# cristianpjensen/thesis-pai-reconstruction

Measured on AMD Instinct MI355X. Metric: train images/sec (256x256, bs=64) Pix2Pix step, higher is better.
Workload: dtype bf16; 1 GPU; Pix2Pix generator+PatchGAN GAN step, 256x256x1 pairs, 64 images/GPU (BASELINE configs[1]); global_batch=64, per_gpu_batch=64, loss_type=gan, parallelism=dp1, grad_bucket_dtype=f32

## Files before the change

include/pai_hip.h:

```cpp
#ifndef PAI_HIP_H
#define PAI_HIP_H

#include <stdint.h>

#ifdef __cplusplus
extern "C" {
#endif

#define PAI_F32 0
#define PAI_BF16 1
#define PAI_U8 2

#define PAI_ACT_NONE 0
#define PAI_ACT_LRELU 1
#define PAI_ACT_RELU 2
#define PAI_ACT_TANH 3
#define PAI_ACT_SILU 4

const char* pai_last_error(void);
int pai_version(void);
int pai_build_flags(void);
int pai_device_info(int* cu_count, int* lds_bytes, char* arch_name, int arch_name_len);

#define PAI_TUNABLE_UNSET (-2147483647 - 1)
// ... 32 lines not shown
int pai_handle_set_wgrad_workspace(void* handle, void* device_memory, int64_t bytes);

int pai_set_workspace(void* zeroed_device_memory, int64_t bytes);
int64_t pai_conv_workspace_bytes(const pai_conv_desc* d, int op);
int pai_set_scratch(void* device_memory, int64_t bytes);
int64_t pai_conv_scratch_bytes(const pai_conv_desc* d, int op);
int pai_set_wgrad_workspace(void* device_memory, int64_t bytes);
int64_t pai_conv_wgrad_workspace_bytes(const pai_conv_desc* d);

int pai_conv_fwd(const pai_conv_desc* d, const void* x1, const void* x2, const void* w_fwd,
                 const float* bias, void* y_raw, void* y_act, float* y_f32, float* stats,
                 void* stream);

int pai_conv_dgrad(const pai_conv_desc* d, const void* dy, const void* w_dgrad, void* dx1,
                   void* dx2, int only_c2, void* stream);

int pai_conv_dgrad_act(const pai_conv_desc* d, const void* dy, const void* w_dgrad, void* dx1,
                       void* dx2, const void* a1, int act1, void* stream);

typedef struct pai_bwd_epilogue {
    const void* z;
    const void* add;
    const float* scale;
    const float* shift;
    const float* mean;
    const float* rstd;
    float* partials;
    int32_t act1, act2;
} pai_bwd_epilogue;
int pai_conv_dgrad_bn_rows_max(const pai_conv_desc* d);
// ... 118 lines not shown
int pai_gate_apply_bwd(int dtype, const void* dout, const void* x, const float* att, const float* logit,
                       int64_t M, int C, const float* mean_a, const float* rstd_a, void* dx_skip, float* dl,
                       float* partials, int relu_out, void* stream);
int pai_gate_hidden_bwd(int dtype, const float* dl, const float* logit, const void* h, const void* ig,
                        const void* sg, int64_t M, int K, const float* mean_a, const float* rstd_a,
                        const float* gamma_a, const float* sums_a, const float* w_a, const float* mean_i,
                        const float* rstd_i, const float* mean_s, const float* rstd_s, void* dsum,
                        float* partials_i, float* partials_s, float* dw_a, float* db_a, void* stream);

int pai_bce_logits(const float* logits, int64_t numel, float target, float loss_scale,
                   double* loss, float grad_scale, float* grad, void* stream);
int pai_l1(const float* pred, const float* target, int64_t numel, float loss_scale, double* loss,
           float grad_scale, float* grad, void* stream);
int pai_mse(const float* pred, const float* target, int64_t numel, float loss_scale, double* loss,
            float grad_scale, float* grad, void* stream);
int pai_scalar_take(double* acc, float* out, void* stream);
int pai_metrics_take(double* sums, int64_t n_images, int64_t numel, float* out3, void* stream);
int pai_tanh_bwd(int dtype, const float* pred, const float* g_a, const float* g_b, int64_t numel,
                 void* dh, void* stream);

int pai_denormalize(const float* x, const float* grad_out_or_null, int64_t numel, float* out,
                    void* stream);

int pai_ssim_sse(const float* pred, const float* target, int NC, int H, int W, int denorm,
                 double* out2, double* per_image, float* full_map, void* stream);
int pai_ssim_psnr_bwd(const float* pred, const float* target, int NC, int H, int W, int denorm,
                      float w_ssim, float w_psnr, const double* sse, float* grad, float* workspace,
                      void* stream);
int64_t pai_ssim_bwd_workspace_floats(int NC, int H, int W);
int pai_eval_planes(const float* pred, const float* target, int NC, int H, int W, int denorm,
// ... 90 lines not shown
```

thesis-pai-reconstruction_amd/build.py:

```python
from __future__ import annotations

import os
import subprocess
import sys
from concurrent.futures import ThreadPoolExecutor

HERE = os.path.dirname(os.path.abspath(__file__))
CSRC = os.path.join(HERE, "csrc")
LIB = os.path.join(HERE, "libpai_hip.so")
STAMPS = os.path.join(CSRC, ".build_stamps.json")
SOURCES = ["api.hip", "gg_simt.hip", "gg_mfma.hip", "gg_wg3.hip", "gg_thin.hip", "gg_small.hip", "gg_group.hip", "gg_pw.hip", "bn.hip", "ew_stream.hip", "gate.hip", "resnet.hip", "inorm.hip", "vit.hip", "loss.hip", "ssim.hip", "eval.hip", "misc.hip", "comm.hip", "plan.hip", "data.hip", "palette.hip", "film_norm.hip"]
HEADERS = [os.path.join(CSRC, "common.h"), os.path.join(CSRC, "plan.h"), os.path.join(CSRC, "gg_tile.h"), os.path.join(HERE, "..", "include", "pai_hip.h")]
FLAGS = ["-O3", "--offload-arch=gfx950", "-fPIC", "-std=c++17", "-Wall", "-Wno-unused-function",
         "-fno-gpu-rdc", "-mllvm", "-amdgpu-mfma-vgpr-form=1"]
EXTRA_FLAGS = {"gg_mfma.hip": ["-fno-slp-vectorize"]}


def _hipcc():
    for c in (os.environ.get("HIPCC"), "/opt/rocm/bin/hipcc", "hipcc"):
        if c and (os.path.isabs(c) and os.path.exists(c) or not os.path.isabs(c)):
            return c
    raise RuntimeError("hipcc not found")


def _digest(paths, extra=""):
    import hashlib
# ... 58 lines not shown
```

thesis-pai-reconstruction_amd/csrc/api.hip:

```cpp
#include <stdarg.h>

#include "common.h"

static thread_local char g_err[512] = "";

void pai_set_error(const char* fmt, ...) {
    va_list ap;
    va_start(ap, fmt);
    vsnprintf(g_err, sizeof(g_err), fmt, ap);
    va_end(ap);
}

extern "C" const char* pai_last_error(void) { return g_err; }
extern "C" int pai_version(void) { return 139; }

extern "C" int pai_build_flags(void) { return 0; }

extern "C" int pai_device_info(int* cu_count, int* lds_bytes, char* arch_name, int arch_name_len) {
    int dev = 0;
    hipError_t e = hipGetDevice(&dev);
    PAI_CHECK(e == hipSuccess, "hipGetDevice: %s", hipGetErrorString(e));
    hipDeviceProp_t p;
    e = hipGetDeviceProperties(&p, dev);
    PAI_CHECK(e == hipSuccess, "hipGetDeviceProperties: %s", hipGetErrorString(e));
    if (cu_count) *cu_count = p.multiProcessorCount;
    if (lds_bytes) *lds_bytes = (int)p.sharedMemPerBlock;
    if (arch_name && arch_name_len > 0) {
        strncpy(arch_name, p.gcnArchName, arch_name_len - 1);
        arch_name[arch_name_len - 1] = 0;
// ... 560 lines not shown
extern "C" int pai_conv_dgrad(const pai_conv_desc* d, const void* dy, const void* w_dgrad,
                              void* dx1, void* dx2, int only_c2, void* stream) {
    GG g;
    if (gg_build_dgrad(d, &g)) return 1;
    PAI_CHECK(dy && w_dgrad, "pai_conv_dgrad: null dy / w");
    PAI_CHECK(only_c2 ? (dx2 && d->C2 > 0) : (dx1 != nullptr), "pai_conv_dgrad: missing output");
    PAI_CHECK(d->C2 == 0 || dx2, "pai_conv_dgrad: C2 > 0 but dx2 is null");
    FwdArgs a;
    memset(&a, 0, sizeof(a));
    a.x1 = dy; a.w = w_dgrad;
    a.y1 = dx1; a.y2 = dx2;
    a.skip_d1 = only_c2;
    return run_fwd(d->dtype, g, a, (hipStream_t)stream);
}

extern "C" int pai_conv_dgrad_act(const pai_conv_desc* d, const void* dy, const void* w_dgrad,
                                  void* dx1, void* dx2, const void* a1, int act1, void* stream) {
    GG g;
    if (gg_build_dgrad(d, &g)) return 1;
    PAI_CHECK(dy && w_dgrad && dx1 && a1, "pai_conv_dgrad_act: null pointer");
    PAI_CHECK(d->C2 == 0 || dx2, "pai_conv_dgrad_act: C2 > 0 but dx2 is null");
    PAI_CHECK(act1 == PAI_ACT_LRELU || act1 == PAI_ACT_RELU || act1 == PAI_ACT_NONE, "pai_conv_dgrad_act: act1=%d", act1);
    FwdArgs a;
    memset(&a, 0, sizeof(a));
    a.x1 = dy; a.w = w_dgrad;
    a.y1 = dx1; a.y2 = dx2;
    hipStream_t s = (hipStream_t)stream;
    FwdPick p = pick_fwd(d->dtype, g, a);
    const bool fused = p.fused || p.k == FK_HEAD_DGRAD;
    if (fused) {
// ... 179 lines not shown
```

thesis-pai-reconstruction_amd/csrc/common.h:

```cpp
#pragma once
#include <hip/hip_runtime.h>
#include <stdint.h>
#include <stdio.h>
#include <string.h>

#include "../../include/pai_hip.h"
#include "plan.h"

typedef unsigned short bf16_t;

void pai_set_error(const char* fmt, ...);

#define PAI_CHECK(cond, ...)                 \
    do {                                     \
        if (!(cond)) {                       \
            pai_set_error(__VA_ARGS__);      \
            return 1;                        \
        }                                    \
    } while (0)

#define PAI_LAUNCH_CHECK()                                              \
    do {                                                                \
        hipError_t e_ = hipGetLastError();                              \
        if (e_ != hipSuccess) {                                         \
// ... 209 lines not shown
int small_rows(const GG& g);
int launch_small(const GG& g, const FwdArgs& a, hipStream_t s);
bool grouped3_ok(int dtype, const GG& g, const FwdArgs& a);
int grouped3_rows(const GG& g);
int launch_grouped3(const GG& g, const FwdArgs& a, hipStream_t s);

bool thin_fwd_ok(int dtype, const GG& g, const FwdArgs& a);
bool thin_dgrad_ok(int dtype, const GG& g, const FwdArgs& a);
bool thin_dgrad_shape_ok(int dtype, const GG& g);
int64_t thin_dgrad_scratch_bytes(const GG& g, const FwdArgs& a);
int launch_thin_fwd(const GG& g, const FwdArgs& a, hipStream_t s);
bool head_dgrad_ok(int dtype, const GG& g, const FwdArgs& a);
int launch_head_dgrad(const GG& g, const FwdArgs& a, hipStream_t s);
int thin_fwd_bwd_rows(int dtype, const GG& g, const FwdArgs& a, int act1, const void* add, const float* scale);
int launch_thin_dgrad(const GG& g, const FwdArgs& a, hipStream_t s);

struct WgradArgs {
    const void *x1, *x2, *dy;
    float* dw;
    float* dbias;
    int overwrite;
    int overwrite_bias;
    float* slab;
    const float *pscale, *pshift;
    int pact;
};
float* wgrad_slab_acquire(int64_t bytes);
int launch_wgrad_slab_sum(float* dw, const float* slab, int nsplits, int64_t n, int overwrite, hipStream_t s);
bool grouped3_wgrad_ok(int dtype, const GG& g, const float* dbias);
int64_t grouped3_wgrad_part_bytes(const GG& g);
// ... 24 lines not shown
```

thesis-pai-reconstruction_amd/csrc/gg_thin.hip:

```cpp
#include "common.h"

#ifndef THIN_ABL
#define THIN_ABL 0
#endif
typedef __attribute__((ext_vector_type(8))) __bf16 bf8_t;
typedef __attribute__((ext_vector_type(4))) __bf16 bf4_t;
typedef __attribute__((ext_vector_type(4))) float f4_t;
typedef __attribute__((ext_vector_type(8))) short s8_t;
typedef __attribute__((ext_vector_type(8))) unsigned short us8_t;

__device__ uint4 g_zero_line_thin[16];


__device__ __forceinline__ bf8_t relu8(bf8_t f) {
    s8_t x = __builtin_bit_cast(s8_t, f);
    const s8_t z = {0, 0, 0, 0, 0, 0, 0, 0};
    return __builtin_bit_cast(bf8_t, __builtin_elementwise_max(x, z));
}

template <int S>
__device__ __forceinline__ us8_t thin_gather8(__amdgpu_buffer_rsrc_t rs, int e0, int ix0, int TW, bool valid) {
    typedef __attribute__((ext_vector_type(4))) unsigned u4_t;
    const int base = ix0 & ~1, o = ix0 & 1;
    const bool neg = valid && e0 + base < 0;
// ... 714 lines not shown
        const int oyl = i >> 5, oxl = i & 31;
        const int oy = 2 * ty0 + oyl, ox = 2 * tx0 + oxl;
        const int ph = (oyl & 1) * 2 + (oxl & 1);
        const int hy0 = (oyl >> 1) + 1, hx0 = (oxl >> 1) + 1;
        const size_t o = ((size_t)n * g.OH + oy) * g.OW + ox;
#pragma unroll
        for (int tt = 0; tt < T; ++tt) {
            const int t = t0 + tt;
            float v = a.bias ? a.bias[t] : 0.f;
#pragma unroll
            for (int k = 0; k < 4; ++k) {
                const int e = tab[ph][k];
                const int hy = hy0 + (int)(signed char)(e & 0xff), hx = hx0 + (int)(signed char)((e >> 8) & 0xff);
                v += Ys[tt][hy * TU_HW + hx][(e >> 16) & 0xff];
            }
            if (t < g.D1) {
                if (a.y1 && !a.skip_d1) ((bf16_t*)a.y1)[o * g.D1 + t] = f2bf(v);
            } else if (a.y2) {
                ((bf16_t*)a.y2)[o * g.D2 + (t - g.D1)] = f2bf(v);
            }
            if (a.yact || a.yf32) {
                const float av = act_apply(v, a.eact);
                if (a.yact) ((bf16_t*)a.yact)[o * g.Cout + t] = f2bf(av);
                if (a.yf32) a.yf32[o * g.Cout + t] = av;
            }
        }
    }
}

static bool thin_up_ok(const GG& g) {
    return pai_tunable("thin_up", 1) && g.nphase == 4 && g.ntaps == 4 && g.OS == 2 && g.wtaps == 16 && (g.H % 16) == 0 &&
           (g.W % 16) == 0 && (g.Cin == 64 || g.Cin == 128);
}

int launch_thin_dgrad(const GG& g, const FwdArgs& a, hipStream_t s) {
    const int T = thin_dgrad_T(g, a);
    const int t0 = (g.Cout == 2 && a.skip_d1) ? 1 : 0;
    if (thin_up_ok(g)) {
        const int tx = g.W / 16, ty = g.H / 16;
        const dim3 grid(g.N * tx * ty);
        if (T == 1 && g.Cin == 128) PAI_LAUNCH((thin_up_k<1, 4>), grid, dim3(256), 0, s, g, a, t0, tx, ty);
        else if (T == 1) PAI_LAUNCH((thin_up_k<1, 2>), grid, dim3(256), 0, s, g, a, t0, tx, ty);
        else if (g.Cin == 128) PAI_LAUNCH((thin_up_k<2, 4>), grid, dim3(256), 0, s, g, a, t0, tx, ty);
        else PAI_LAUNCH((thin_up_k<2, 2>), grid, dim3(256), 0, s, g, a, t0, tx, ty);
        PAI_LAUNCH_CHECK();
        return 0;
    }
// ... 416 lines not shown
```

thesis-pai-reconstruction_amd/engine.py:

```python
from __future__ import annotations

import os
from typing import Callable, List, Optional

import torch
import torch.nn as nn

from . import ops
from .ops import ACT_LRELU, ACT_NONE, ACT_RELU, ACT_TANH

BN_EPS_DEFAULT = 1e-5


def _fwd_pack_strides(mod) -> tuple:
    if isinstance(mod, nn.ConvTranspose2d):
        cin, cout, kh, kw = mod.weight.shape
        return (1, kh * kw * cin, kw * cin, cin)
    cout, cin, kh, kw = mod.weight.shape
    return (kh * kw * cin, 1, kw * cin, cin)


def _strides_match(t: torch.Tensor, want: tuple) -> bool:
    return all(s == w or n == 1 for s, w, n in zip(t.stride(), want, t.shape))

# ... 759 lines not shown
        S["logits"] = torch.empty(N, 1, P["oh"], P["ow"], dtype=torch.float32, device=device)
        S["grads"] = None
        return S

    def release(self, S):
        S["P"]["free"].append(S)

    def _to_nhwc(self, t, dst, dtype):
        t = t.to(torch.float32)
        t = t.contiguous() if t.shape[1] == 1 else t.permute(0, 2, 3, 1).contiguous()
        if dtype == torch.float32:
            return t.reshape(-1)
        ops.cast(t, dst)
        return dst

    def forward(self, x, y, dtype, y2=None):
        if not (x.is_cuda and y.is_cuda):
            raise ops.PaiError("Discriminator (HIP) needs HIP device tensors; there is no CPU path")
        N, C, H, W = x.shape
        if C != self.in_ch or y.shape != x.shape or (y2 is not None and y2.shape != x.shape):
            raise ops.PaiError(f"Discriminator expects [N,{self.in_ch},H,W] tensors of one shape, got {tuple(x.shape)} "
                               f"and {tuple(y.shape)}")
        reps = 1 if y2 is None else 2
        S = self.acquire(N * reps, H, W, dtype, x.device)
        P = S["P"]
        if y2 is None and dtype != torch.float32 and C == 1:
            ops.cast_multi([(x.detach().to(torch.float32).contiguous().reshape(-1), S["x"]),
                            (y.detach().to(torch.float32).contiguous().reshape(-1), S["y"])])
            S["xin"], S["yin"] = S["x"], S["y"]
        elif y2 is None:
            S["xin"] = self._to_nhwc(x, S["x"], dtype)
# ... 1 lines not shown
        else:
            half = N * H * W * C
            pairs = []
            for src, dst in ((x, S["x"][:half]), (x, S["x"][half:]), (y, S["y"][:half]), (y2, S["y"][half:])):
                t = src.detach().to(torch.float32)
                t = t.contiguous() if C == 1 else t.permute(0, 2, 3, 1).contiguous()
                pairs.append((t.reshape(-1), dst))
            ops.cast_multi(pairs)
            S["xin"], S["yin"] = S["x"], S["y"]
        refresh_packs(self.packs, dtype)
        wf, _ = self.packs[0].get(dtype)
        ops.conv_fwd(P["desc"][0], S["xin"], S["yin"], wf, self.convs[0].bias, y_act=S["a"][0])
        for k in range(1, 4):
            wf, _ = self.packs[k].get(dtype)
            ops.conv_fwd(P["desc"][k], S["a"][k - 1], None, wf, self.convs[k].bias, y_act=S["a"][k])
        wf, _ = self.packs[4].get(dtype)
        S["logits"] = torch.empty_like(S["logits"])
        ops.conv_fwd(P["desc"][4], S["a"][3], None, wf, None, y_f32=S["logits"])
        return S["logits"], S

    def _wgrad_desc(self, P, k):
        if os.environ.get("PAI_D_WGRAD_SOLO", "1") in ("", "0"):
            return P["desc"][k]
        solo = P.setdefault("desc_solo", {})
        if k not in solo:
            import copy
            d = copy.copy(P["desc"][k])
            d.hints = 1
            solo[k] = d
        return solo[k]

    def backward(self, S, glogits, need_params: bool, need_dy: bool, fresh: bool = False):
        conv_wgrad = ops.conv_wgrad_overwrite_w if fresh else ops.conv_wgrad
        P = S["P"]
        N, H, W, dtype, dev = P["N"], P["H"], P["W"], P["dtype"], P["device"]
        if S["grads"] is None:
            G = {"du": [torch.empty_like(a) for a in S["a"]],
                 "dl": torch.empty(S["logits"].numel(), dtype=dtype, device=dev),
                 "dy": torch.empty(N * H * W * self.in_ch, dtype=dtype, device=dev)}
            S["grads"] = G
        G = S["grads"]
        A = self.arena() if need_params else None
        hook = self.grad_ready_hook
        glogits = glogits.contiguous().float()
        if dtype == torch.float32:
            dl = glogits.reshape(-1)
        else:
            ops.cast(glogits, G["dl"])
            dl = G["dl"]
        d = P["desc"][4]
        side = self._side
        if need_params:
            with torch.cuda.stream(side.fork(d)):
                ops.conv_wgrad(d, S["a"][3], None, dl, A.seg(self.convs[4].weight), None)
                if hook is not None:
                    hook(A, A.end_of(self.convs[4].weight))
            side.mark_scratch()
        _, wd = self.packs[4].get(dtype)
        ops.conv_dgrad_act(d, dl, wd, G["du"][3], None, S["a"][3], ACT_LRELU)
        for k in range(3, -1, -1):
            conv = self.convs[k]
            d = P["desc"][k]
            if need_params and k == 0:
                with torch.cuda.stream(side.fork_tail()):
                    (ops.conv_wgrad if min(_cin_cout(conv)) <= 2 else conv_wgrad)(
                        d, S["xin"], S["yin"], G["du"][0], A.seg(conv.weight), A.seg(conv.bias))
            elif need_params:
                with torch.cuda.stream(side.fork(d)):
                    conv_wgrad(self._wgrad_desc(P, k), S["a"][k - 1], None, G["du"][k], A.seg(conv.weight), A.seg(conv.bias))
                    if hook is not None:
                        hook(A, A.end_of(conv.bias))
            if k > 0:
                _, wd = self.packs[k].get(dtype)
                ops.conv_dgrad_act(d, G["du"][k], wd, G["du"][k - 1], None, S["a"][k - 1], ACT_LRELU)
            elif need_dy:
                _, wd = self.packs[0].get(dtype)
                ops.conv_dgrad(d, G["du"][0], wd, None, G["dy"], only_c2=True)
        side.join()
        if need_params and hook is not None:
            hook(A, A.end_of(self.convs[0].bias))
        if not need_dy:
            return None
        gy = torch.empty(N * H * W * self.in_ch, dtype=torch.float32, device=dev)
        ops.cast(G["dy"], gy)
        if self.in_ch == 1:
            return gy.view(N, 1, H, W)
        return gy.view(N, H, W, self.in_ch).permute(0, 3, 1, 2)
```

thesis-pai-reconstruction_amd/functional.py:

```python
from __future__ import annotations

import math

import torch

from . import ops


class _SlotRef:

    def __init__(self, engine, slot):
        self.engine, self.slot = engine, slot

    def take(self):
        if self.slot is None:
            raise ops.PaiError("second backward through the same forward: the engine's activation slot has already "
                               "been consumed (retain_graph is not supported)")
        slot, self.slot = self.slot, None
        return slot

    def __del__(self):
        if self.slot is not None:
            try:
                self.engine.release(self.slot)
# ... 71 lines not shown
        else:
            engine.release(slot)
        return logits

    @staticmethod
    def backward(ctx, glogits):
        engine, slot, params = ctx.engine, ctx.ref.take(), ctx.params
        arena = engine.arena()
        fresh = arena.begin_backward(params, overwrite_weights=True)
        engine.backward(slot, glogits, True, False, fresh)
        arena.attach(params)
        engine.release(slot)
        return (None,) * (5 + len(params))


class DiscGenLossFunction(torch.autograd.Function):

    @staticmethod
    def forward(ctx, x, pred, target, engine, dtype, l1_weight, *params):
        _check_f32_cuda(x, pred, target)
        if ctx.needs_input_grad[0] or ctx.needs_input_grad[2]:
            raise ops.PaiError("gradient w.r.t. the conditioning image / the target is not supported")
        logits, slot = engine.forward(x, pred, dtype)
        pc, tc = pred.contiguous().float(), target.contiguous().float()
        need_pred, need_params = ctx.needs_input_grad[1], any(ctx.needs_input_grad[6:])
        need = need_pred or need_params
        gl = torch.empty_like(logits) if need else None
        gp = torch.empty_like(pc) if need_pred else None
        ent = _ACC.get(pc.device, "gan_g")
        ops.bce_logits(logits, 1.0, 1.0, ent[0], 1.0, gl)
        ops.l1(pc, tc, float(l1_weight), ent[0], float(l1_weight), gp)
        out = torch.empty((), dtype=torch.float32, device=pc.device)
        ops.scalar_take(ent[0], out)
        _ACC.taken(ent)
        if need:
            ctx.engine, ctx.ref, ctx.params = engine, _SlotRef(engine, slot), params
            ctx.need_pred, ctx.need_params = need_pred, need_params
            ctx.save_for_backward(*[g for g in (gl, gp) if g is not None])
        else:
            engine.release(slot)
        return out

    @staticmethod
    def backward(ctx, gout):
        engine, slot, params = ctx.engine, ctx.ref.take(), ctx.params
        saved = list(ctx.saved_tensors)
        gl = _scaled(saved.pop(0), gout)
        fresh = False
        if ctx.need_params:
            arena = engine.arena()
            fresh = arena.begin_backward(params, overwrite_weights=True)
        gy = engine.backward(slot, gl, ctx.need_params, ctx.need_pred, fresh)
        if ctx.need_params:
            arena.attach(params)
        engine.release(slot)
        if ctx.need_pred:
            gp = _scaled(saved.pop(0), gout)
            if gy.is_contiguous() and gy.numel() % 8 == 0:
                ops.add_act(torch.float32, gy, gp, ops.ACT_NONE, gy)
            else:
                gy = gy + gp
        return (None, gy, None, None, None, None) + (None,) * len(params)


def _check_f32_cuda(*ts):
    for t in ts:
        if not t.is_cuda:
            raise ops.PaiError("pai losses/metrics need HIP device tensors (no CPU fallback exists)")


class _MeanLoss(torch.autograd.Function):
# ... 39 lines not shown
        ent[1] = False


_ACC = _Accumulators()


_UNIT = {}


def unit_seed(device) -> torch.Tensor:
    t = _UNIT.get(device.index)
    if t is None:
        t = torch.ones((), dtype=torch.float32, device=device)
        _UNIT[device.index] = t
    return t


def _scaled(grad, gout):
    u = _UNIT.get(gout.device.index) if gout.is_cuda else None
    if u is not None and gout.data_ptr() == u.data_ptr():
        return grad
    return grad * gout


class _GanDiscLoss(torch.autograd.Function):

    @staticmethod
    def forward(ctx, labels, n_real):
        _check_f32_cuda(labels)
        x = labels.contiguous().float()
# ... 324 lines not shown
```

thesis-pai-reconstruction_amd/lib.py:

```python
from __future__ import annotations

import ctypes as C
import os

HERE = os.path.dirname(os.path.abspath(__file__))
LIB_PATH = os.environ.get("PAI_HIP_LIB") or os.path.join(HERE, "libpai_hip.so")

F32, BF16 = 0, 1
U8 = 2
ACT_NONE, ACT_LRELU, ACT_RELU, ACT_TANH = 0, 1, 2, 3
ACT_SILU = 4
HINT_SOLO = 1


class PaiError(RuntimeError):
    pass


class ConvDesc(C.Structure):
    _fields_ = [("dtype", C.c_int32), ("transposed", C.c_int32),
                ("N", C.c_int32), ("H", C.c_int32), ("W", C.c_int32),
                ("C1", C.c_int32), ("C2", C.c_int32), ("Cout", C.c_int32),
                ("kernel", C.c_int32), ("stride", C.c_int32), ("pad", C.c_int32),
                ("relu1", C.c_int32), ("relu2", C.c_int32), ("epilogue_act", C.c_int32),
# ... 33 lines not shown
    "pai_conv_out_hw": (_I, [_D, C.POINTER(_I), C.POINTER(_I)]),
    "pai_conv_fwd_stats_rows": (_I, [_D]),
    "pai_conv_fwd_stats_rows_max": (_I, [_D]),
    "pai_bn_stats_buffer_rows": (_I, [_I]),
    "pai_conv_kernel_id": (_I, [_D, _I]),
    "pai_conv_kernel_name": (_I, [_D, _I, C.c_char_p, _I]),
    "pai_set_workspace": (_I, [_P, _L]),
    "pai_conv_workspace_bytes": (_L, [_D, _I]),
    "pai_set_scratch": (_I, [_P, _L]),
    "pai_conv_scratch_bytes": (_L, [_D, _I]),
    "pai_set_wgrad_workspace": (_I, [_P, _L]),
    "pai_conv_wgrad_workspace_bytes": (_L, [_D]),
    "pai_conv_fwd": (_I, [_D, _P, _P, _P, _P, _P, _P, _P, _P, _P]),
    "pai_conv_dgrad": (_I, [_D, _P, _P, _P, _P, _I, _P]),
    "pai_conv_dgrad_act": (_I, [_D, _P, _P, _P, _P, _P, _I, _P]),
    "pai_conv_dgrad_bn_rows_max": (_I, [_D]),
    "pai_conv_dgrad_bn": (_I, [_D, _P, _P, _P, _P, C.POINTER(BwdEpilogue), C.POINTER(_I), _P]),
    "pai_bn_bwd_finalize": (_I, [_P, _I, _I, _P, _P, _P, _P]),
    "pai_conv_fwd_bn": (_I, [_D, _P, _P, _P, _P, _P, _P, _I, C.POINTER(BnTrain), _P, _P]),
    "pai_conv_dgrad_bn_apply": (_I, [_D, _P, _P, _P, _P, C.POINTER(BwdEpilogue), _P, _P, _P, _P, _P, _P]),
    "pai_conv_bn_fused": (_I, [_D, _I]),
    "pai_conv_wgrad": (_I, [_D, _P, _P, _P, _P, _P, _P]),
    "pai_conv_wgrad_overwrite": (_I, [_D, _P, _P, _P, _P, _P, _P]),
    "pai_conv_wgrad_overwrite_w": (_I, [_D, _P, _P, _P, _P, _P, _P]),
    "pai_conv_prologue_ok": (_I, [_D]),
    "pai_conv_fwd_pro": (_I, [_D, _P, _P, _P, _P, _P, _P, _P, _I, _P]),
    "pai_conv_wgrad_pro": (_I, [_D, _P, _P, _P, _P, _I, _P, _P, _I, _P]),
    "pai_pack_weights": (_I, [_I, _P, _I, _I, _I, _P, _P, _P]),
    "pai_build_flags": (_I, []),
    "pai_pack_weights_multi": (_I, [_I, _P, _P, _P, _P, _P, _P, _P]),
# ... 130 lines not shown
```

thesis-pai-reconstruction_amd/models/wrapper.py:

```python
from typing import Literal

import torch
import torch.nn as nn

from .. import functional as PF
from .. import ops
from ..engine import DiscEngine
from ..lightning import LightningModule
from .utils import denormalize, init_weights, psnr, rmse, ssim

L1_WEIGHT = 50


class UnetWrapper(LightningModule):

    def __init__(self, unet: nn.Module,
                 loss_type: Literal["gan", "ssim", "psnr", "ssim+psnr", "mse"] = "gan"):
        super().__init__()
        self.automatic_optimization = False
        self.unet = unet
        self.loss_type = loss_type
        self.reuse_generator_forward = True

        self.discriminator = None
# ... 73 lines not shown
        metrics_early = None

        if self.loss_type == "gan":
            opt_d = self.optimizers()[1]
            if reuse:
                self.unet.bn_updates_per_forward = 2
                try:
                    pred_g = self.unet(x)
                finally:
                    self.unet.bn_updates_per_forward = 1

                metrics_early = self._metrics_async(pred_g, target)

            self.toggle_optimizer(opt_d)
            pred = pred_g.detach() if reuse else self.unet(x)
            if getattr(self.discriminator, "supports_batched_pairs", False):
                n = x.shape[0]
                labels = self.discriminator.forward_pairs(x, target, pred)
                d_loss = PF.gan_discriminator_loss_pairs(labels, n)
            else:
                target_label = self.discriminator(x, target)
                pred_label = self.discriminator(x, pred)
                d_loss = self.discriminator_loss(pred_label, target_label)
            self.log("d_loss", d_loss, prog_bar=True)
            self.discriminator.zero_grad(set_to_none=True)
            self._arm(opt_d)
            self.manual_backward(d_loss)
            opt_d.step()
            self.untoggle_optimizer(opt_d)

        opt_g = self.optimizers()
# ... 54 lines not shown
            h = nnops.ConvK4S2.apply(h, conv.weight, conv.bias, ACT_NONE, dtype)
            h = nnops.InstanceNormAct.apply(h, float(norm.eps), ACT_LRELU)
        else:
            h = nnops.ConvK4S2.apply(h, conv.weight, conv.bias, ACT_LRELU, dtype)
        return h.float().permute(0, 3, 1, 2)


class Discriminator(nn.Module):

    def __init__(self, in_channels: int = 3):
        super().__init__()
        self.in_channels = in_channels
        self.compute_dtype = torch.float32
        self.supports_batched_pairs = True
        self.supports_fused_generator_loss = True
        self.discriminator = nn.Sequential(
            DiscriminatorBlock(in_channels * 2, 64, norm=False),
            DiscriminatorBlock(64, 128),
            DiscriminatorBlock(128, 256),
            DiscriminatorBlock(256, 512),
            nn.Conv2d(512, 1, kernel_size=4, padding=1, bias=False),
        )
        self._engine = None

    @property
    def engine(self) -> DiscEngine:
        if self._engine is None:
            object.__setattr__(self, "_engine", DiscEngine(self))
        return self._engine

    def forward(self, x, y):
        eng = self.engine
        params = [p for p, _ in eng.ordered_params()]
        return PF.DiscFunction.apply(x, y, eng, self.compute_dtype, *params)

    def generator_loss(self, x, y, target, l1_weight):
        eng = self.engine
        params = [p for p, _ in eng.ordered_params()]
        return PF.DiscGenLossFunction.apply(x, y, target, eng, self.compute_dtype, float(l1_weight), *params)

    def forward_pairs(self, x, y_real, y_fake):
        eng = self.engine
        params = [p for p, _ in eng.ordered_params()]
        return PF.DiscPairsFunction.apply(x.detach(), y_real.detach(), y_fake.detach(), eng, self.compute_dtype, *params)
```

thesis-pai-reconstruction_amd/ops.py:

```python
from __future__ import annotations

import ctypes as C

import threading
from typing import Optional

import torch

from . import lib as L
from .lib import ACT_LRELU, ACT_NONE, ACT_RELU, ACT_SILU, ACT_TANH, BF16, F32, U8, ConvDesc, PaiError


def code_of(dtype: torch.dtype) -> int:
    if dtype == torch.float32:
        return F32
    if dtype == torch.bfloat16:
        return BF16
    raise PaiError(f"unsupported storage dtype {dtype}")


_TLS = threading.local()


def _stream():
# ... 271 lines not shown
        L.check(L.load().pai_conv_wgrad_pro(C.byref(d), _p(x1), _p(dy), _p(dw, torch.float32), _p(dbias, torch.float32),
                                            int(overwrite), _p(pre_scale, torch.float32), _p(pre_shift, torch.float32),
                                            int(pre_act), _stream()), "pai_conv_wgrad_pro")


def conv_dgrad(d, dy, w_dgrad, dx1, dx2=None, only_c2=False):
    with _Timed(d, 1):
        L.check(L.load().pai_conv_dgrad(C.byref(d), _p(dy), _p(w_dgrad), _p(dx1), _p(dx2), int(only_c2),
                                        _stream()), "pai_conv_dgrad")


def conv_dgrad_act(d, dy, w_dgrad, dx1, dx2, a1, act1):
    with _Timed(d, 1):
        L.check(L.load().pai_conv_dgrad_act(C.byref(d), _p(dy), _p(w_dgrad), _p(dx1), _p(dx2), _p(a1), int(act1),
                                            _stream()), "pai_conv_dgrad_act")


def conv_dgrad_bn_rows_max(d) -> int:
    return L.load().pai_conv_dgrad_bn_rows_max(C.byref(d))


def conv_dgrad_bn(d, dy, w_dgrad, dx1, dx2, z, act1, add=None, act2=ACT_NONE, scale=None, shift=None,
                  mean=None, rstd=None, partials=None) -> int:
    e = L.BwdEpilogue(_p(z), _p(add), _p(scale, torch.float32), _p(shift, torch.float32), _p(mean, torch.float32),
                      _p(rstd, torch.float32), _p(partials, torch.float32), int(act1), int(act2))
    rows = C.c_int(0)
    with _Timed(d, 1):
        L.check(L.load().pai_conv_dgrad_bn(C.byref(d), _p(dy), _p(w_dgrad), _p(dx1), _p(dx2), C.byref(e),
                                           C.byref(rows), _stream()), "pai_conv_dgrad_bn")
    return rows.value
# ... 761 lines not shown
```

Before: 11470 images/s.

## Fuse discriminator head conv, BCE loss, and head dgrad into one kernel

```diff
diff --git a/include/pai_hip.h b/include/pai_hip.h
--- a/include/pai_hip.h
+++ b/include/pai_hip.h
@@ -70,6 +70,10 @@
 
 int pai_conv_dgrad(const pai_conv_desc* d, const void* dy, const void* w_dgrad, void* dx1,
                    void* dx2, int only_c2, void* stream);
+
+int pai_conv_dgrad_f32add_ok(const pai_conv_desc* d);
+int pai_conv_dgrad_f32add(const pai_conv_desc* d, const void* dy, const void* w_dgrad, const float* addend,
+                          float* dx2_f32, void* stream);
 
 int pai_conv_dgrad_act(const pai_conv_desc* d, const void* dy, const void* w_dgrad, void* dx1,
                        void* dx2, const void* a1, int act1, void* stream);
@@ -218,6 +222,10 @@
            float grad_scale, float* grad, void* stream);
 int pai_mse(const float* pred, const float* target, int64_t numel, float loss_scale, double* loss,
             float grad_scale, float* grad, void* stream);
+int pai_head_loss_ok(const pai_conv_desc* d, int has_bias);
+int pai_head_loss(const pai_conv_desc* d, const void* a3, const void* w_fwd, const void* w_dgrad, int n_first,
+                  float target_first, float target_rest, float loss_scale, double* loss, float grad_scale,
+                  float* logits, void* dl, float* dl_f32, void* du, const void* act_src, int act, void* stream);
 int pai_scalar_take(double* acc, float* out, void* stream);
 int pai_metrics_take(double* sums, int64_t n_images, int64_t numel, float* out3, void* stream);
 int pai_tanh_bwd(int dtype, const float* pred, const float* g_a, const float* g_b, int64_t numel,
diff --git a/thesis-pai-reconstruction_amd/build.py b/thesis-pai-reconstruction_amd/build.py
--- a/thesis-pai-reconstruction_amd/build.py
+++ b/thesis-pai-reconstruction_amd/build.py
@@ -9,7 +9,7 @@
 CSRC = os.path.join(HERE, "csrc")
 LIB = os.path.join(HERE, "libpai_hip.so")
 STAMPS = os.path.join(CSRC, ".build_stamps.json")
-SOURCES = ["api.hip", "gg_simt.hip", "gg_mfma.hip", "gg_wg3.hip", "gg_thin.hip", "gg_small.hip", "gg_group.hip", "gg_pw.hip", "bn.hip", "ew_stream.hip", "gate.hip", "resnet.hip", "inorm.hip", "vit.hip", "loss.hip", "ssim.hip", "eval.hip", "misc.hip", "comm.hip", "plan.hip", "data.hip", "palette.hip", "film_norm.hip"]
+SOURCES = ["api.hip", "gg_simt.hip", "gg_mfma.hip", "gg_wg3.hip", "gg_thin.hip", "head.hip", "gg_small.hip", "gg_group.hip", "gg_pw.hip", "bn.hip", "ew_stream.hip", "gate.hip", "resnet.hip", "inorm.hip", "vit.hip", "loss.hip", "ssim.hip", "eval.hip", "misc.hip", "comm.hip", "plan.hip", "data.hip", "palette.hip", "film_norm.hip"]
 HEADERS = [os.path.join(CSRC, "common.h"), os.path.join(CSRC, "plan.h"), os.path.join(CSRC, "gg_tile.h"), os.path.join(HERE, "..", "include", "pai_hip.h")]
 FLAGS = ["-O3", "--offload-arch=gfx950", "-fPIC", "-std=c++17", "-Wall", "-Wno-unused-function",
          "-fno-gpu-rdc", "-mllvm", "-amdgpu-mfma-vgpr-form=1"]
diff --git a/thesis-pai-reconstruction_amd/csrc/api.hip b/thesis-pai-reconstruction_amd/csrc/api.hip
--- a/thesis-pai-reconstruction_amd/csrc/api.hip
+++ b/thesis-pai-reconstruction_amd/csrc/api.hip
@@ -12,7 +12,7 @@
 }
 
 extern "C" const char* pai_last_error(void) { return g_err; }
-extern "C" int pai_version(void) { return 139; }
+extern "C" int pai_version(void) { return 140; }
 
 extern "C" int pai_build_flags(void) { return 0; }
 
@@ -603,6 +603,26 @@
     return run_fwd(d->dtype, g, a, (hipStream_t)stream);
 }
 
+extern "C" int pai_conv_dgrad_f32add_ok(const pai_conv_desc* d) {
+    GG g;
+    if (!d || gg_build_dgrad(d, &g)) return 0;
+    return pai_tunable("head_fused", 1) && thin_up_f32add_ok(d->dtype, g) ? 1 : 0;
+}
+
+extern "C" int pai_conv_dgrad_f32add(const pai_conv_desc* d, const void* dy, const void* w_dgrad, const float* addend,
+                                     float* dx2_f32, void* stream) {
+    GG g;
+    if (gg_build_dgrad(d, &g)) return 1;
+    PAI_CHECK(dy && w_dgrad && addend && dx2_f32, "pai_conv_dgrad_f32add: null pointer");
+    PAI_CHECK(thin_up_f32add_ok(d->dtype, g), "pai_conv_dgrad_f32add: not a bf16 (1 | 1)-channel k4 s2 layer on thin_up_k (ask pai_conv_dgrad_f32add_ok)");
+    FwdArgs a;
+    memset(&a, 0, sizeof(a));
+    a.x1 = dy; a.w = w_dgrad;
+    a.yf32 = dx2_f32; a.badd = addend;
+    a.skip_d1 = 1;
+    return launch_thin_dgrad(g, a, (hipStream_t)stream);
+}
+
 extern "C" int pai_conv_dgrad_act(const pai_conv_desc* d, const void* dy, const void* w_dgrad,
                                   void* dx1, void* dx2, const void* a1, int act1, void* stream) {
     GG g;
diff --git a/thesis-pai-reconstruction_amd/csrc/common.h b/thesis-pai-reconstruction_amd/csrc/common.h
--- a/thesis-pai-reconstruction_amd/csrc/common.h
+++ b/thesis-pai-reconstruction_amd/csrc/common.h
@@ -247,6 +247,7 @@
 int launch_head_dgrad(const GG& g, const FwdArgs& a, hipStream_t s);
 int thin_fwd_bwd_rows(int dtype, const GG& g, const FwdArgs& a, int act1, const void* add, const float* scale);
 int launch_thin_dgrad(const GG& g, const FwdArgs& a, hipStream_t s);
+bool thin_up_f32add_ok(int dtype, const GG& g);
 
 struct WgradArgs {
     const void *x1, *x2, *dy;
diff --git a/thesis-pai-reconstruction_amd/csrc/gg_thin.hip b/thesis-pai-reconstruction_amd/csrc/gg_thin.hip
--- a/thesis-pai-reconstruction_amd/csrc/gg_thin.hip
+++ b/thesis-pai-reconstruction_amd/csrc/gg_thin.hip
@@ -752,6 +752,13 @@
                 const int hy = hy0 + (int)(signed char)(e & 0xff), hx = hx0 + (int)(signed char)((e >> 8) & 0xff);
                 v += Ys[tt][hy * TU_HW + hx][(e >> 16) & 0xff];
             }
+            if (a.badd) {
+                if (t >= g.D1) {
+                    const size_t idx = o * g.D2 + (t - g.D1);
+                    a.yf32[idx] = bf2f(f2bf(v)) + ((const float*)a.badd)[idx];
+                }
+                continue;
+            }
             if (t < g.D1) {
                 if (a.y1 && !a.skip_d1) ((bf16_t*)a.y1)[o * g.D1 + t] = f2bf(v);
             } else if (a.y2) {
@@ -769,6 +776,10 @@
 static bool thin_up_ok(const GG& g) {
     return pai_tunable("thin_up", 1) && g.nphase == 4 && g.ntaps == 4 && g.OS == 2 && g.wtaps == 16 && (g.H % 16) == 0 &&
            (g.W % 16) == 0 && (g.Cin == 64 || g.Cin == 128);
+}
+
+bool thin_up_f32add_ok(int dtype, const GG& g) {
+    return thin_dgrad_shape_ok(dtype, g) && thin_up_ok(g) && g.Cout == 2 && g.D1 == 1 && g.D2 == 1;
 }
 
 int launch_thin_dgrad(const GG& g, const FwdArgs& a, hipStream_t s) {
diff --git a/thesis-pai-reconstruction_amd/csrc/head.hip b/thesis-pai-reconstruction_amd/csrc/head.hip
--- /dev/null
+++ b/thesis-pai-reconstruction_amd/csrc/head.hip
@@ -0,0 +1,209 @@
+#include "common.h"
+
+typedef __attribute__((ext_vector_type(8))) __bf16 bf8_t;
+typedef __attribute__((ext_vector_type(4))) float f4_t;
+
+constexpr int HL_THREADS = 512, HL_WAVES = HL_THREADS / 64;
+constexpr int HL_LD = 17;
+constexpr int64_t HL_LDS_MAX = 96 * 1024;
+
+struct HeadLoss {
+    const bf16_t* a3;
+    const bf16_t* wf;
+    const bf16_t* wd;
+    float* logits;
+    bf16_t* dl;
+    float* dl32;
+    bf16_t* du;
+    const bf16_t* act_src;
+    double* loss;
+    int N, H, W, C, OH, OW;
+    int n_first;
+    float t_first, t_rest;
+    double ls_first, ls_rest;
+    float gs_first, gs_rest;
+    int act;
+    int rg;
+    int xcd;
+};
+
+static int64_t head_loss_lds_bytes(int H, int W, int C, bool with_du) {
+    const int64_t ys = (((int64_t)H * W * HL_LD * 4) + 15) & ~(int64_t)15;
+    const int64_t dls = (((int64_t)(H - 1) * (W - 1) * 4) + 15) & ~(int64_t)15;
+    return ys + dls + (with_du ? (int64_t)16 * C * 2 : 0);
+}
+
+template <int KS>
+__global__ __launch_bounds__(HL_THREADS) void head_loss_k(HeadLoss p) {
+    extern __shared__ __attribute__((aligned(16))) unsigned char hl_sm[];
+    __shared__ double wsum[HL_WAVES];
+    const int P = p.H * p.W, Q = p.OH * p.OW;
+    float* Ys = (float*)hl_sm;
+    float* dls = (float*)(hl_sm + ((((size_t)P * HL_LD * 4) + 15) & ~(size_t)15));
+    bf16_t* wt = (bf16_t*)((unsigned char*)dls + ((((size_t)Q * 4) + 15) & ~(size_t)15));
+    const int tid = threadIdx.x, lane = tid & 63, wid = tid >> 6;
+    const int fr = lane & 15, fq = lane >> 4;
+    int n, rg;
+    if (p.xcd) {
+        n = (blockIdx.x & 7) + 8 * (blockIdx.x / (8 * p.rg));
+        rg = (blockIdx.x >> 3) % p.rg;
+    } else {
+        n = blockIdx.x / p.rg;
+        rg = blockIdx.x - n * p.rg;
+    }
+    const bool first = n < p.n_first;
+    const float tconst = first ? p.t_first : p.t_rest;
+    const float gscale = first ? p.gs_first : p.gs_rest;
+
+    if (p.du) {
+        for (int i = tid; i < p.C * 16; i += HL_THREADS) {
+            const int c = i >> 4, t = i & 15;
+            wt[t * p.C + c] = p.wd[i];
+        }
+    }
+    bf8_t af[KS];
+#pragma unroll
+    for (int s = 0; s < KS; ++s) af[s] = *(const bf8_t*)(p.wf + (size_t)fr * p.C + 32 * s + 8 * fq);
+    const bf16_t* x = p.a3 + (size_t)n * P * p.C;
+    for (int p0 = wid * 16; p0 < P; p0 += HL_WAVES * 16) {
+        const int m = min(p0 + fr, P - 1);
+        bf8_t bfr[KS];
+#pragma unroll
+        for (int s = 0; s < KS; ++s) bfr[s] = *(const bf8_t*)(x + (size_t)m * p.C + 32 * s + 8 * fq);
+        f4_t acc = (f4_t){0.f, 0.f, 0.f, 0.f};
+#pragma unroll
+        for (int s = 0; s < KS; ++s) acc = __builtin_amdgcn_mfma_f32_16x16x32_bf16(af[s], bfr[s], acc, 0, 0, 0);
+        if (p0 + fr < P) {
+#pragma unroll
+            for (int r = 0; r < 4; ++r) Ys[(p0 + fr) * HL_LD + 4 * fq + r] = acc[r];
+        }
+    }
+    __syncthreads();
+    double lsum = 0.0;
+    for (int i = tid; i < Q; i += HL_THREADS) {
+        const int oy = i / p.OW, ox = i - oy * p.OW;
+        float v = 0.f;
+#pragma unroll
+        for (int k = 0; k < 16; ++k) {
+            const int iy = oy + (k >> 2) - 1, ix = ox + (k & 3) - 1;
+            if ((unsigned)iy < (unsigned)p.H && (unsigned)ix < (unsigned)p.W) v += Ys[(iy * p.W + ix) * HL_LD + k];
+        }
+        const float xv = v;
+        const float l = fmaxf(xv, 0.f) - xv * tconst + log1pf(expf(-fabsf(xv)));
+        const float g = 1.f / (1.f + expf(-xv)) - tconst;
+        const float gs = g * gscale;
+        const bf16_t gb = f2bf(gs);
+        dls[i] = bf2f(gb);
+        lsum += (double)l;
+        if (rg == 0) {
+            const size_t o = (size_t)n * Q + i;
+            p.logits[o] = xv;
+            if (p.dl) p.dl[o] = gb;
+            if (p.dl32) p.dl32[o] = gs;
+        }
+    }
+    if (rg == 0) {
+        double v = lsum * (first ? p.ls_first : p.ls_rest);
+#pragma unroll
+        for (int o = 32; o > 0; o >>= 1) v += __shfl_xor(v, o, 64);
+        if (lane == 0) wsum[wid] = v;
+    }
+    __syncthreads();
+    if (rg == 0 && tid == 0) {
+        double v = wsum[0];
+#pragma unroll
+        for (int w = 1; w < HL_WAVES; ++w) v += wsum[w];
+        if (fabs(v) < 256.0) v = rint(v * 0x1p36) * 0x1p-36;
+        atomicAdd(p.loss, v);
+    }
+    if (!p.du) return;
+    const int r0 = (p.H * rg) / p.rg, r1 = (p.H * (rg + 1)) / p.rg;
+    const int groups = p.C / 8;
+    const int items = (r1 - r0) * p.W * groups;
+    for (int item = tid; item < items; item += HL_THREADS) {
+        const int pix = item / groups, cg = item - pix * groups;
+        const int ry = pix / p.W, ox = pix - ry * p.W, oy = r0 + ry;
+        float acc[8];
+#pragma unroll
+        for (int j = 0; j < 8; ++j) acc[j] = 0.f;
+#pragma unroll
+        for (int t = 0; t < 16; ++t) {
+            const int sy = oy + 1 - (t >> 2), sx = ox + 1 - (t & 3);
+            if ((unsigned)sy >= (unsigned)p.OH || (unsigned)sx >= (unsigned)p.OW) continue;
+            const float v = dls[sy * p.OW + sx];
+            float wv[8];
+            V8<bf16_t>::ld(wt + t * p.C + cg * 8, wv);
+#pragma unroll
+            for (int j = 0; j < 8; ++j) acc[j] = fmaf(v, wv[j], acc[j]);
+        }
+        const size_t o = ((size_t)n * P + (size_t)oy * p.W + ox) * p.C + cg * 8;
+        float zv[8];
+        V8<bf16_t>::ld(p.act_src + o, zv);
+#pragma unroll
+        for (int j = 0; j < 8; ++j) {
+            const float gq = bf2f(f2bf(acc[j]));
+            acc[j] = p.act == PAI_ACT_NONE ? gq : gq * act_grad(zv[j], p.act);
+        }
+        V8<bf16_t>::st(p.du + o, acc);
+    }
+}
+
+static bool head_loss_shape_ok(const pai_conv_desc* d, int has_bias) {
+    if (!d || has_bias || d->dtype != PAI_BF16 || d->transposed || d->kernel != 4 || d->stride != 1 || d->pad != 1) return false;
+    if (d->Cout != 1 || d->C2 != 0 || d->relu1 || d->epilogue_act != PAI_ACT_NONE || d->groups > 1) return false;
+    if (d->N <= 0 || d->H < 2 || d->W < 2 || (d->C1 % 32) != 0) return false;
+    const int ks = d->C1 / 32;
+    if (!(ks == 1 || ks == 2 || ks == 4 || ks == 8 || ks == 16)) return false;
+    return head_loss_lds_bytes(d->H, d->W, d->C1, true) <= HL_LDS_MAX;
+}
+
+extern "C" int pai_head_loss_ok(const pai_conv_desc* d, int has_bias) {
+    return pai_tunable("head_fused", 1) && head_loss_shape_ok(d, has_bias) ? 1 : 0;
+}
+
+extern "C" int pai_head_loss(const pai_conv_desc* d, const void* a3, const void* w_fwd, const void* w_dgrad, int n_first,
+                             float target_first, float target_rest, float loss_scale, double* loss, float grad_scale,
+                             float* logits, void* dl, float* dl_f32, void* du, const void* act_src, int act, void* stream) {
+    PAI_CHECK(head_loss_shape_ok(d, 0), "pai_head_loss: not a bias-free bf16 k4 s1 p1 C -> 1 head within the LDS bound (ask pai_head_loss_ok)");
+    PAI_CHECK(a3 && w_fwd && loss && logits, "pai_head_loss: null pointer");
+    PAI_CHECK(!du || (w_dgrad && act_src), "pai_head_loss: du needs w_dgrad and act_src");
+    PAI_CHECK(act == PAI_ACT_LRELU || act == PAI_ACT_RELU || act == PAI_ACT_NONE, "pai_head_loss: act=%d", act);
+    HeadLoss p;
+    memset(&p, 0, sizeof(p));
+    p.a3 = (const bf16_t*)a3; p.wf = (const bf16_t*)w_fwd; p.wd = (const bf16_t*)w_dgrad;
+    p.logits = logits; p.dl = (bf16_t*)dl; p.dl32 = dl_f32; p.du = (bf16_t*)du; p.act_src = (const bf16_t*)act_src;
+    p.loss = loss;
+    p.N = d->N; p.H = d->H; p.W = d->W; p.C = d->C1; p.OH = d->H - 1; p.OW = d->W - 1;
+    p.n_first = n_first < 0 ? 0 : (n_first > d->N ? d->N : n_first);
+    p.t_first = target_first; p.t_rest = target_rest;
+    const int64_t per = (int64_t)p.OH * p.OW, nf = per * p.n_first, nr = per * (p.N - p.n_first);
+    if (nf > 0) { p.ls_first = (double)loss_scale / (double)nf; p.gs_first = (float)((double)grad_scale / (double)nf); }
+    if (nr > 0) { p.ls_rest = (double)loss_scale / (double)nr; p.gs_rest = (float)((double)grad_scale / (double)nr); }
+    p.act = act;
+    int rg = du ? pai_tunable("head_loss_rg", 4) : 1;
+    if (rg < 1) rg = 1;
+    if (rg > p.H) rg = p.H;
+    p.rg = rg;
+    p.xcd = (p.N % 8) == 0 ? 1 : 0;
+    const size_t lds = (size_t)head_loss_lds_bytes(p.H, p.W, p.C, du != nullptr);
+    const dim3 grid((unsigned)(p.N * rg));
+    hipStream_t s = (hipStream_t)stream;
+#define HL_CASE(KK)                                                                                                     \
+    case KK: {                                                                                                          \
+        static PerDeviceOnce attr;                                                                                      \
+        if (attr.first()) {                                                                                             \
+            const hipError_t e = hipFuncSetAttribute(reinterpret_cast<const void*>(&head_loss_k<KK>),                   \
+                                                     hipFuncAttributeMaxDynamicSharedMemorySize, (int)HL_LDS_MAX);      \
+            PAI_CHECK(e == hipSuccess, "pai_head_loss: hipFuncSetAttribute(max dynamic LDS): %s", hipGetErrorString(e)); \
+        }                                                                                                               \
+        PAI_LAUNCH(head_loss_k<KK>, grid, dim3(HL_THREADS), lds, s, p);                                                 \
+        break;                                                                                                          \
+    }
+    switch (p.C / 32) {
+        HL_CASE(1) HL_CASE(2) HL_CASE(4) HL_CASE(8) HL_CASE(16)
+        default: PAI_CHECK(false, "pai_head_loss: unsupported C %d", p.C);
+    }
+#undef HL_CASE
+    PAI_LAUNCH_CHECK();
+    return 0;
+}
diff --git a/thesis-pai-reconstruction_amd/engine.py b/thesis-pai-reconstruction_amd/engine.py
--- a/thesis-pai-reconstruction_amd/engine.py
+++ b/thesis-pai-reconstruction_amd/engine.py
@@ -797,7 +797,7 @@
         ops.cast(t, dst)
         return dst
 
-    def forward(self, x, y, dtype, y2=None):
+    def forward(self, x, y, dtype, y2=None, head: bool = True):
         if not (x.is_cuda and y.is_cuda):
             raise ops.PaiError("Discriminator (HIP) needs HIP device tensors; there is no CPU path")
         N, C, H, W = x.shape
@@ -829,10 +829,45 @@
         for k in range(1, 4):
             wf, _ = self.packs[k].get(dtype)
             ops.conv_fwd(P["desc"][k], S["a"][k - 1], None, wf, self.convs[k].bias, y_act=S["a"][k])
+        S["head_done"] = False
+        if not head:
+            return None, S
         wf, _ = self.packs[4].get(dtype)
         S["logits"] = torch.empty_like(S["logits"])
         ops.conv_fwd(P["desc"][4], S["a"][3], None, wf, None, y_f32=S["logits"])
         return S["logits"], S
+
+    @staticmethod
+    def fused_enabled() -> bool:
+        return os.environ.get("PAI_HEAD_FUSED", "1") not in ("", "0")
+
+    def head_fused_ok(self, dtype) -> bool:
+        return dtype == torch.bfloat16 and self.fused_enabled() and self.convs[4].bias is None
+
+    def _grads(self, S):
+        if S["grads"] is None:
+            P = S["P"]
+            S["grads"] = {"du": [torch.empty_like(a) for a in S["a"]],
+                          "dl": torch.empty(S["logits"].numel(), dtype=P["dtype"], device=P["device"]),
+                          "dl32": torch.empty(S["logits"].numel(), dtype=torch.float32, device=P["device"]),
+                          "dy": torch.empty(P["N"] * P["H"] * P["W"] * self.in_ch, dtype=P["dtype"], device=P["device"])}
+        return S["grads"]
+
+    def forward_loss(self, x, y, dtype, y2, n_first, target_first, target_rest, acc, need_grad: bool):
+        if not (x.is_cuda and y.is_cuda):
+            raise ops.PaiError("Discriminator (HIP) needs HIP device tensors; there is no CPU path")
+        N = x.shape[0] * (1 if y2 is None else 2)
+        P = self._plan(N, x.shape[2], x.shape[3], dtype, x.device)
+        if not ops.head_loss_ok(P["desc"][4], self.convs[4].bias is not None):
+            return None
+        _, S = self.forward(x, y, dtype, y2=y2, head=False)
+        wf, wd = self.packs[4].get(dtype)
+        G = self._grads(S) if need_grad else None
+        ops.head_loss(P["desc"][4], S["a"][3], wf, wd if need_grad else None, n_first, target_first, target_rest, 1.0, acc, 1.0,
+                      S["logits"], G["dl"] if need_grad else None, G["dl32"] if need_grad else None,
+                      G["du"][3] if need_grad else None, ACT_LRELU)
+        S["head_done"] = need_grad
+        return S
 
     def _wgrad_desc(self, P, k):
         if os.environ.get("PAI_D_WGRAD_SOLO", "1") in ("", "0"):
@@ -845,26 +880,28 @@
             solo[k] = d
         return solo[k]
 
-    def backward(self, S, glogits, need_params: bool, need_dy: bool, fresh: bool = False):
+    def backward(self, S, glogits, need_params: bool, need_dy: bool, fresh: bool = False, head_done: bool = False,
+                 addend=None):
         conv_wgrad = ops.conv_wgrad_overwrite_w if fresh else ops.conv_wgrad
         P = S["P"]
         N, H, W, dtype, dev = P["N"], P["H"], P["W"], P["dtype"], P["device"]
-        if S["grads"] is None:
-            G = {"du": [torch.empty_like(a) for a in S["a"]],
-                 "dl": torch.empty(S["logits"].numel(), dtype=dtype, device=dev),
-                 "dy": torch.empty(N * H * W * self.in_ch, dtype=dtype, device=dev)}
-            S["grads"] = G
-        G = S["grads"]
+        G = self._grads(S)
         A = self.arena() if need_params else None
         hook = self.grad_ready_hook
-        glogits = glogits.contiguous().float()
-        if dtype == torch.float32:
-            dl = glogits.reshape(-1)
+        if head_done:
+            if not S.get("head_done"):
+                raise ops.PaiError("DiscEngine.backward(head_done=True) without a forward_loss that kept its gradients")
+            dl = G["dl"]
         else:
-            ops.cast(glogits, G["dl"])
-            dl = G["dl"]
+            glogits = glogits.contiguous().float()
+            if dtype == torch.float32:
+                dl = glogits.reshape(-1)
+            else:
+                ops.cast(glogits, G["dl"])
+                dl = G["dl"]
         d = P["desc"][4]
         side = self._side
+        gy = None
         if need_params:
             with torch.cuda.stream(side.fork(d)):
                 ops.conv_wgrad(d, S["a"][3], None, dl, A.seg(self.convs[4].weight), None)
@@ -872,7 +909,8 @@
                     hook(A, A.end_of(self.convs[4].weight))
             side.mark_scratch()
         _, wd = self.packs[4].get(dtype)
-        ops.conv_dgrad_act(d, dl, wd, G["du"][3], None, S["a"][3], ACT_LRELU)
+        if not head_done:
+            ops.conv_dgrad_act(d, dl, wd, G["du"][3], None, S["a"][3], ACT_LRELU)
         for k in range(3, -1, -1):
             conv = self.convs[k]
             d = P["desc"][k]
@@ -890,14 +928,25 @@
                 ops.conv_dgrad_act(d, G["du"][k], wd, G["du"][k - 1], None, S["a"][k - 1], ACT_LRELU)
             elif need_dy:
                 _, wd = self.packs[0].get(dtype)
-                ops.conv_dgrad(d, G["du"][0], wd, None, G["dy"], only_c2=True)
+                if addend is not None and self.in_ch == 1 and self.fused_enabled() and addend.dtype == torch.float32 \
+                        and addend.is_contiguous() and addend.numel() == N * H * W and ops.conv_dgrad_f32add_ok(d):
+                    gy = torch.empty(N * H * W, dtype=torch.float32, device=dev)
+                    ops.conv_dgrad_f32add(d, G["du"][0], wd, addend, gy)
+                else:
+                    ops.conv_dgrad(d, G["du"][0], wd, None, G["dy"], only_c2=True)
         side.join()
         if need_params and hook is not None:
             hook(A, A.end_of(self.convs[0].bias))
         if not need_dy:
             return None
+        if gy is not None:
+            return gy.view(N, 1, H, W)
         gy = torch.empty(N * H * W * self.in_ch, dtype=torch.float32, device=dev)
         ops.cast(G["dy"], gy)
-        if self.in_ch == 1:
-            return gy.view(N, 1, H, W)
-        return gy.view(N, H, W, self.in_ch).permute(0, 3, 1, 2)
+        gy = gy.view(N, 1, H, W) if self.in_ch == 1 else gy.view(N, H, W, self.in_ch).permute(0, 3, 1, 2)
+        if addend is not None:
+            if gy.is_contiguous() and gy.numel() % 8 == 0:
+                ops.add_act(torch.float32, gy, addend, ops.ACT_NONE, gy)
+            else:
+                gy = gy + addend
+        return gy
diff --git a/thesis-pai-reconstruction_amd/functional.py b/thesis-pai-reconstruction_amd/functional.py
--- a/thesis-pai-reconstruction_amd/functional.py
+++ b/thesis-pai-reconstruction_amd/functional.py
@@ -109,6 +109,52 @@
         return (None,) * (5 + len(params))
 
 
+class DiscPairsLossFunction(torch.autograd.Function):
+
+    @staticmethod
+    def forward(ctx, x, y_real, y_fake, engine, dtype, *params):
+        _check_f32_cuda(x, y_real, y_fake)
+        if ctx.needs_input_grad[0] or ctx.needs_input_grad[1] or ctx.needs_input_grad[2]:
+            raise ops.PaiError("DiscPairsLossFunction carries no gradient to its image inputs; detach them")
+        need = any(ctx.needs_input_grad[5:])
+        n = x.shape[0]
+        ent = _ACC.get(x.device, "gan_d")
+        out = torch.empty((), dtype=torch.float32, device=x.device)
+        slot = engine.forward_loss(x, y_real, dtype, y_fake, n, 1.0, 0.0, ent[0], need) if engine.head_fused_ok(dtype) else None
+        ctx.fused = slot is not None
+        grad = None
+        if slot is None:
+            logits, slot = engine.forward(x, y_real, dtype, y2=y_fake)
+            flat = logits.view(-1)
+            k = (flat.numel() // logits.shape[0]) * n
+            grad = torch.empty_like(flat) if need else None
+            ops.bce_logits(flat[:k], 1.0, 1.0, ent[0], 1.0, grad[:k] if need else None)
+            ops.bce_logits(flat[k:], 0.0, 1.0, ent[0], 1.0, grad[k:] if need else None)
+        ops.scalar_take(ent[0], out)
+        _ACC.taken(ent)
+        if need:
+            ctx.engine, ctx.ref, ctx.params = engine, _SlotRef(engine, slot), params
+            if grad is not None:
+                ctx.save_for_backward(grad)
+        else:
+            engine.release(slot)
+        return out
+
+    @staticmethod
+    def backward(ctx, gout):
+        engine, slot, params = ctx.engine, ctx.ref.take(), ctx.params
+        arena = engine.arena()
+        fresh = arena.begin_backward(params, overwrite_weights=True)
+        if ctx.fused and _is_unit(gout):
+            engine.backward(slot, None, True, False, fresh, head_done=True)
+        else:
+            grad = slot["grads"]["dl32"] if ctx.fused else ctx.saved_tensors[0]
+            engine.backward(slot, _scaled(grad, gout).view(slot["logits"].shape), True, False, fresh)
+        arena.attach(params)
+        engine.release(slot)
+        return (None,) * (5 + len(params))
+
+
 class DiscGenLossFunction(torch.autograd.Function):
 
     @staticmethod
@@ -116,14 +162,18 @@
         _check_f32_cuda(x, pred, target)
         if ctx.needs_input_grad[0] or ctx.needs_input_grad[2]:
             raise ops.PaiError("gradient w.r.t. the conditioning image / the target is not supported")
-        logits, slot = engine.forward(x, pred, dtype)
         pc, tc = pred.contiguous().float(), target.contiguous().float()
         need_pred, need_params = ctx.needs_input_grad[1], any(ctx.needs_input_grad[6:])
         need = need_pred or need_params
-        gl = torch.empty_like(logits) if need else None
         gp = torch.empty_like(pc) if need_pred else None
         ent = _ACC.get(pc.device, "gan_g")
-        ops.bce_logits(logits, 1.0, 1.0, ent[0], 1.0, gl)
+        slot = engine.forward_loss(x, pred, dtype, None, x.shape[0], 1.0, 1.0, ent[0], need) if engine.head_fused_ok(dtype) else None
+        ctx.fused = slot is not None
+        gl = None
+        if slot is None:
+            logits, slot = engine.forward(x, pred, dtype)
+            gl = torch.empty_like(logits) if need else None
+            ops.bce_logits(logits, 1.0, 1.0, ent[0], 1.0, gl)
         ops.l1(pc, tc, float(l1_weight), ent[0], float(l1_weight), gp)
         out = torch.empty((), dtype=torch.float32, device=pc.device)
         ops.scalar_take(ent[0], out)
@@ -140,16 +190,24 @@
     def backward(ctx, gout):
         engine, slot, params = ctx.engine, ctx.ref.take(), ctx.params
         saved = list(ctx.saved_tensors)
-        gl = _scaled(saved.pop(0), gout)
+        unit = _is_unit(gout)
+        head_done = ctx.fused and unit
+        if head_done:
+            gl = None
+        elif ctx.fused:
+            gl = _scaled(slot["grads"]["dl32"], gout).view(slot["logits"].shape)
+        else:
+            gl = _scaled(saved.pop(0), gout)
         fresh = False
         if ctx.need_params:
             arena = engine.arena()
             fresh = arena.begin_backward(params, overwrite_weights=True)
-        gy = engine.backward(slot, gl, ctx.need_params, ctx.need_pred, fresh)
+        addend = saved[0] if ctx.need_pred and unit and engine.fused_enabled() else None
+        gy = engine.backward(slot, gl, ctx.need_params, ctx.need_pred, fresh, head_done=head_done, addend=addend)
         if ctx.need_params:
             arena.attach(params)
         engine.release(slot)
-        if ctx.need_pred:
+        if ctx.need_pred and addend is None:
             gp = _scaled(saved.pop(0), gout)
             if gy.is_contiguous() and gy.numel() % 8 == 0:
                 ops.add_act(torch.float32, gy, gp, ops.ACT_NONE, gy)
@@ -219,6 +277,11 @@
         t = torch.ones((), dtype=torch.float32, device=device)
         _UNIT[device.index] = t
     return t
+
+
+def _is_unit(gout) -> bool:
+    u = _UNIT.get(gout.device.index) if gout.is_cuda else None
+    return u is not None and gout.data_ptr() == u.data_ptr()
 
 
 def _scaled(grad, gout):
diff --git a/thesis-pai-reconstruction_amd/lib.py b/thesis-pai-reconstruction_amd/lib.py
--- a/thesis-pai-reconstruction_amd/lib.py
+++ b/thesis-pai-reconstruction_amd/lib.py
@@ -71,6 +71,10 @@
     "pai_conv_fwd": (_I, [_D, _P, _P, _P, _P, _P, _P, _P, _P, _P]),
     "pai_conv_dgrad": (_I, [_D, _P, _P, _P, _P, _I, _P]),
     "pai_conv_dgrad_act": (_I, [_D, _P, _P, _P, _P, _P, _I, _P]),
+    "pai_conv_dgrad_f32add_ok": (_I, [_D]),
+    "pai_conv_dgrad_f32add": (_I, [_D, _P, _P, _P, _P, _P]),
+    "pai_head_loss_ok": (_I, [_D, _I]),
+    "pai_head_loss": (_I, [_D, _P, _P, _P, _I, _F, _F, _F, _P, _F, _P, _P, _P, _P, _P, _I, _P]),
     "pai_conv_dgrad_bn_rows_max": (_I, [_D]),
     "pai_conv_dgrad_bn": (_I, [_D, _P, _P, _P, _P, C.POINTER(BwdEpilogue), C.POINTER(_I), _P]),
     "pai_bn_bwd_finalize": (_I, [_P, _I, _I, _P, _P, _P, _P]),
diff --git a/thesis-pai-reconstruction_amd/models/wrapper.py b/thesis-pai-reconstruction_amd/models/wrapper.py
--- a/thesis-pai-reconstruction_amd/models/wrapper.py
+++ b/thesis-pai-reconstruction_amd/models/wrapper.py
@@ -111,7 +111,9 @@
 
             self.toggle_optimizer(opt_d)
             pred = pred_g.detach() if reuse else self.unet(x)
-            if getattr(self.discriminator, "supports_batched_pairs", False):
+            if pred.is_cuda and getattr(self.discriminator, "supports_fused_pairs_loss", False):
+                d_loss = self.discriminator.pairs_loss(x, target, pred)
+            elif getattr(self.discriminator, "supports_batched_pairs", False):
                 n = x.shape[0]
                 labels = self.discriminator.forward_pairs(x, target, pred)
                 d_loss = PF.gan_discriminator_loss_pairs(labels, n)
@@ -196,6 +198,7 @@
         self.compute_dtype = torch.float32
         self.supports_batched_pairs = True
         self.supports_fused_generator_loss = True
+        self.supports_fused_pairs_loss = True
         self.discriminator = nn.Sequential(
             DiscriminatorBlock(in_channels * 2, 64, norm=False),
             DiscriminatorBlock(64, 128),
@@ -225,3 +228,8 @@
         eng = self.engine
         params = [p for p, _ in eng.ordered_params()]
         return PF.DiscPairsFunction.apply(x.detach(), y_real.detach(), y_fake.detach(), eng, self.compute_dtype, *params)
+
+    def pairs_loss(self, x, y_real, y_fake):
+        eng = self.engine
+        params = [p for p, _ in eng.ordered_params()]
+        return PF.DiscPairsLossFunction.apply(x.detach(), y_real.detach(), y_fake.detach(), eng, self.compute_dtype, *params)
diff --git a/thesis-pai-reconstruction_amd/ops.py b/thesis-pai-reconstruction_amd/ops.py
--- a/thesis-pai-reconstruction_amd/ops.py
+++ b/thesis-pai-reconstruction_amd/ops.py
@@ -309,6 +309,29 @@
     with _Timed(d, 1):
         L.check(L.load().pai_conv_dgrad_act(C.byref(d), _p(dy), _p(w_dgrad), _p(dx1), _p(dx2), _p(a1), int(act1),
                                             _stream()), "pai_conv_dgrad_act")
+
+
+def conv_dgrad_f32add_ok(d) -> bool:
+    return bool(L.load().pai_conv_dgrad_f32add_ok(C.byref(d)))
+
+
+def conv_dgrad_f32add(d, dy, w_dgrad, addend, dx2_f32):
+    with _Timed(d, 1):
+        L.check(L.load().pai_conv_dgrad_f32add(C.byref(d), _p(dy), _p(w_dgrad), _p(addend, torch.float32),
+                                               _p(dx2_f32, torch.float32), _stream()), "pai_conv_dgrad_f32add")
+
+
+def head_loss_ok(d, has_bias: bool = False) -> bool:
+    return bool(L.load().pai_head_loss_ok(C.byref(d), int(bool(has_bias))))
+
+
+def head_loss(d, a3, w_fwd, w_dgrad, n_first, target_first, target_rest, loss_scale, loss, grad_scale, logits, dl=None,
+              dl_f32=None, du=None, act=ACT_LRELU):
+    L.check(L.load().pai_head_loss(C.byref(d), _p(a3, torch.bfloat16), _p(w_fwd), _p(w_dgrad), int(n_first),
+                                   float(target_first), float(target_rest), float(loss_scale), _p(loss, torch.float64),
+                                   float(grad_scale), _p(logits, torch.float32), _p(dl, torch.bfloat16),
+                                   _p(dl_f32, torch.float32), _p(du, torch.bfloat16), _p(a3) if du is not None else None,
+                                   int(act), _stream()), "pai_head_loss")
 
 
 def conv_dgrad_bn_rows_max(d) -> int:
```

New measurement: 11610 images/s, median of 6. 1.01x the previous value.
